# Avokadoen/zig_vulkan

Hardware: AMD Instinct MI355X
Metric: Mrays/s at 1920x1080 on 512^3 brickmap (8^3 bricks, primary + shadow, 1 spp); achieved % of HBM roofline (higher is better)
Workload: dtype f32

## Files before the change

### bindings/vrt_hip.zig

```

const std = @import("std");

pub const Ctx = opaque {};
pub const Grid = opaque {};
pub const Vox = opaque {};
pub const Benchmark = opaque {};

pub const Status = enum(c_int) {
    ok = 0,
    invalid_arg = -1,
    oom = -2,
    out_of_range = -3,
    hip = -4,
    no_device = -5,
    state = -6,
    rccl = -7,
    vox_invalid_id = -100,
    vox_expected_size_header = -101,
    vox_expected_xyzi_header = -102,
    vox_expected_rgba_header = -103,
    vox_unexpected_version = -104,
    vox_invalid_file_content = -105,
    vox_multiple_pack_chunks = -106,
    _,
// ... 151 lines not shown

pub const TUNE_NO_SKIP_TO_BOX: u32 = 1 << 0;
pub const TUNE_NO_PATH_BRICK_LDS: u32 = 1 << 1;
pub const TUNE_NO_PATH_HALFBLOCKS: u32 = 1 << 2;
pub const TUNE_PATH_EAGER_START: u32 = 1 << 3;
pub const TUNE_DIST_NO_BROADCAST: u32 = 1 << 4;
pub const TUNE_NO_CELL_OCCUPANCY: u32 = 1 << 5;
pub const TUNE_NO_START_SHORTCUT: u32 = 1 << 6;
pub const TUNE_PATH_AHEAD: u32 = 1 << 7;
pub const TUNE_PATH_DISTANCE: u32 = 1 << 8;
pub const TUNE_NO_PATH_DILATED: u32 = 1 << 9;
pub const TUNE_NO_PATH_GRID_EXIT: u32 = 1 << 10;
pub const TUNE_PATH_BLOCKS64: u32 = 1 << 11;
pub const TUNE_PATH_TWO_AHEAD: u32 = 1 << 12;
pub const TUNE_NO_PATH_POOL: u32 = 1 << 13;
pub const TUNE_NO_SMALL_FRAME_SPLIT: u32 = 1 << 14;
pub const TUNE_NO_BOUNCE_WAVE_GROUPS: u32 = 1 << 15;
pub const TUNE_NO_SAMPLE_UNITS: u32 = 1 << 16;
pub const TUNE_NO_DEFERRED_MATERIAL: u32 = 1 << 17;
pub const TUNE_NO_CELL_MATERIAL: u32 = 1 << 18;
pub const TUNE_GRID_EXIT_ANY_BOX: u32 = 1 << 19;
pub const TUNE_NO_BOUNCE_AUTOTUNE: u32 = 1 << 20;
pub const TUNE_PRESENT_OWN_STREAM: u32 = 1 << 21;

pub const GridConfig = extern struct {
    brick_alloc: u64 = 0,
    base_t: f32 = 0.01,
    min_point: [3]f32 = .{ 0, 0, 0 },
    scale: f32 = 1.0,
    brick_dimension: u32 = 4,
};

pub const CameraConfig = extern struct {
    viewport_height: f32 = 2,
    origin: [3]f32 = .{ 0, 0, 0 },
    samples_per_pixel: i32 = 2,
    max_bounce: i32 = 2,
};

pub const SunConfig = extern struct {
    enabled: u32 = 1,
    color: [3]f32 = .{ 1, 1.1, 1 },
    radius: f32 = 5,
    sun_distance: f32 = 1000,
};

// ... 149 lines not shown
```

### include/vrt_hip.h

```cpp
#ifndef VRT_HIP_H
#define VRT_HIP_H

#include <stdint.h>

#ifdef __cplusplus
extern "C" {
#endif

#define VRT_ABI_VERSION 4u

enum {
    VRT_OK = 0,
    VRT_E_INVALID_ARG = -1,
    VRT_E_OOM = -2,
    VRT_E_OUT_OF_RANGE = -3,
    VRT_E_HIP = -4,
    VRT_E_NO_DEVICE = -5,
    VRT_E_STATE = -6,
    VRT_E_RCCL = -7
};

typedef enum vrt_buffer_id {
    VRT_BUF_GRID_STATE = 0,
    VRT_BUF_MATERIALS = 1,
// ... 68 lines not shown

#define VRT_TUNE_NO_SKIP_TO_BOX     (1u << 0)
#define VRT_TUNE_NO_PATH_BRICK_LDS  (1u << 1)
#define VRT_TUNE_NO_PATH_HALFBLOCKS (1u << 2)
#define VRT_TUNE_PATH_EAGER_START   (1u << 3)
#define VRT_TUNE_DIST_NO_BROADCAST  (1u << 4)
#define VRT_TUNE_NO_CELL_OCCUPANCY  (1u << 5)
#define VRT_TUNE_NO_START_SHORTCUT  (1u << 6)
#define VRT_TUNE_PATH_AHEAD          (1u << 7)
#define VRT_TUNE_PATH_DISTANCE       (1u << 8)
#define VRT_TUNE_NO_PATH_DILATED     (1u << 9)
#define VRT_TUNE_NO_PATH_GRID_EXIT   (1u << 10)
#define VRT_TUNE_PATH_BLOCKS64        (1u << 11)
#define VRT_TUNE_PATH_TWO_AHEAD       (1u << 12)
#define VRT_TUNE_NO_PATH_POOL         (1u << 13)
#define VRT_TUNE_NO_SMALL_FRAME_SPLIT (1u << 14)
#define VRT_TUNE_NO_BOUNCE_WAVE_GROUPS (1u << 15)
#define VRT_TUNE_NO_SAMPLE_UNITS     (1u << 16)
#define VRT_TUNE_NO_DEFERRED_MATERIAL (1u << 17)
#define VRT_TUNE_NO_CELL_MATERIAL     (1u << 18)
#define VRT_TUNE_GRID_EXIT_ANY_BOX    (1u << 19)
#define VRT_TUNE_NO_BOUNCE_AUTOTUNE   (1u << 20)
#define VRT_TUNE_PRESENT_OWN_STREAM   (1u << 21)
#define VRT_TUNE_ALL                0x3FFFFFu

typedef struct vrt_ctx vrt_ctx;

int vrt_create(const vrt_config *cfg, vrt_ctx **out);

void vrt_destroy(vrt_ctx *ctx);

int vrt_upload(vrt_ctx *ctx, vrt_buffer_id id, uint64_t byte_offset, const void *src, uint64_t nbytes);

uint64_t vrt_buffer_size(const vrt_ctx *ctx, vrt_buffer_id id);

int vrt_upload_device(vrt_ctx *ctx, vrt_buffer_id id, uint64_t byte_offset, const void *dev_src, uint64_t nbytes);

int vrt_dispatch(vrt_ctx *ctx, const vrt_camera_device *camera, const vrt_sun_device *sun);
int vrt_wait(vrt_ctx *ctx);

int vrt_reserve_samples(vrt_ctx *ctx, uint32_t max_samples_per_pixel);

int vrt_dispatch_repeat(vrt_ctx *ctx, const vrt_camera_device *camera, const vrt_sun_device *sun, uint32_t frames);

int vrt_dispatch_timed(vrt_ctx *ctx, const vrt_camera_device *camera, const vrt_sun_device *sun, uint32_t frames, float *ms_per_frame);

int vrt_read_rgba8(vrt_ctx *ctx, void *dst, uint64_t nbytes);
// ... 178 lines not shown
```

### zig_vulkan_amd/_lib.py

```python
from __future__ import annotations

import ctypes as C
import os

_HERE = os.path.dirname(os.path.abspath(__file__))
LIB_PATH = os.environ.get("VRT_HIP_LIB") or os.path.join(_HERE, "libvrt_hip.so")

VRT_ABI_VERSION = 4

VRT_OK = 0
VRT_E_INVALID_ARG = -1
VRT_E_OOM = -2
VRT_E_OUT_OF_RANGE = -3
VRT_E_HIP = -4
VRT_E_NO_DEVICE = -5
VRT_E_STATE = -6
VRT_E_RCCL = -7

ERROR_NAMES = {
    VRT_E_INVALID_ARG: "VRT_E_INVALID_ARG",
    VRT_E_OOM: "VRT_E_OOM",
    VRT_E_OUT_OF_RANGE: "VRT_E_OUT_OF_RANGE",
    VRT_E_HIP: "VRT_E_HIP",
    VRT_E_NO_DEVICE: "VRT_E_NO_DEVICE",
    VRT_E_STATE: "VRT_E_STATE",
    VRT_E_RCCL: "VRT_E_RCCL",
}

TUNE_NO_SKIP_TO_BOX, TUNE_NO_PATH_BRICK_LDS, TUNE_NO_PATH_HALFBLOCKS, TUNE_PATH_EAGER_START, TUNE_DIST_NO_BROADCAST = 1, 2, 4, 8, 16
TUNE_NO_CELL_OCCUPANCY, TUNE_NO_START_SHORTCUT, TUNE_PATH_AHEAD, TUNE_PATH_DISTANCE, TUNE_NO_PATH_DILATED, TUNE_NO_PATH_GRID_EXIT, TUNE_PATH_BLOCKS64, TUNE_PATH_TWO_AHEAD = 32, 64, 128, 256, 512, 1024, 2048, 4096
TUNE_NO_SMALL_FRAME_SPLIT = 16384
TUNE_NO_BOUNCE_WAVE_GROUPS = 32768
TUNE_NO_SAMPLE_UNITS = 65536
TUNE_NO_DEFERRED_MATERIAL = 131072
TUNE_NO_CELL_MATERIAL = 262144
TUNE_GRID_EXIT_ANY_BOX = 524288
TUNE_NO_BOUNCE_AUTOTUNE = 1048576
TUNE_PRESENT_OWN_STREAM = 2097152
TUNE_NO_PATH_POOL = 8192

BUF_GRID_STATE, BUF_MATERIALS, BUF_BRICK_STATUS, BUF_BRICK_INDEX, BUF_BRICK_OCCUPANCY, BUF_BRICK_START_INDEX, BUF_MATERIAL_INDEX = range(7)
BUF_COUNT = 7


class VrtError(RuntimeError):
    def __init__(self, code: int, message: str):
        super().__init__(f"{ERROR_NAMES.get(code, code)}: {message}")
        self.code = code


class GridState(C.Structure):
    _fields_ = [
        ("voxel_dim_x", C.c_uint32), ("voxel_dim_y", C.c_uint32), ("voxel_dim_z", C.c_uint32),
        ("dim_x", C.c_uint32), ("dim_y", C.c_uint32), ("dim_z", C.c_uint32),
        ("padding1", C.c_uint32), ("padding2", C.c_uint32),
        ("min_point_base_t", C.c_float * 4),
        ("max_point_scale", C.c_float * 4),
    ]


class Material(C.Structure):
# ... 241 lines not shown
```

### zig_vulkan_amd/csrc/vrt_api.hip

```cpp
#include <hip/hip_runtime.h>
#include <algorithm>
#include <cstdio>
#include <cstdlib>
#include <cstring>
#include <mutex>
#include <new>
#include <string>
#include <thread>
#include "host_brick_grid.hpp"
#include "vrt_ctx.h"

using namespace vrt_impl;

namespace {
thread_local std::string g_create_error;
}

namespace vrt_impl {

int fail(vrt_ctx *ctx, int code, const std::string &msg) {
    if (ctx) ctx->err = msg;
    else g_create_error = msg;
    return code;
}

void free_ctx(vrt_ctx *c) {
    if (!c) return;
    DeviceGuard dg(c->device);
    if (c->stream) (void)hipStreamSynchronize(c->stream);
    query_release(c);
    dist_destroy(c);
    c->res.release_all();
// ... 444 lines not shown
        const bool cnt = cfg->enable_counters != 0;
        if (!c->kernel || !c->kernel_lockstep || !c->kernel_single || !c->kernel_single1 ||
            (cnt && (!c->product[0] || !c->product[1] || !c->product[2]))) {
            free_ctx(c);
#ifdef VRT_DEV_VARIANTS
            return fail(nullptr, VRT_E_INVALID_ARG, "no kernel for this configuration");
#else
            return fail(nullptr, VRT_E_INVALID_ARG, "no kernel for this kernel_variant in the product build of libvrt_hip (development variants: make dev)");
#endif
        }
        auto any_kernel = [&](auto pred) {
            const vrt::KernelFn fns[12] = {c->kernel, c->kernel_lockstep, c->kernel_single, c->kernel_single1, c->product[0], c->product[1], c->product[2],
                                           c->kernel_grid_exit, c->product_grid_exit, c->kernel_grid_exit_path, c->product_grid_exit_path, c->bounce_auto};
            for (vrt::KernelFn fn : fns) {
                const vrt::KernelEntry *e = fn ? vrt::kernel_entry_of(fn) : nullptr;
                if (e && pred(*e)) return true;
            }
            return false;
        };
        if (any_kernel([](const vrt::KernelEntry &e) { return !e.path && e.mode == vrt::kStatusBytes; })) {
            const size_t status_bytes_size = (size_t)((cells + 31u) / 32u) * 32u + 64u;
            VRT_CREATE_HIP(c->res.device(&c->d_status_bytes, status_bytes_size));
            VRT_CREATE_HIP(hipMemsetAsync(c->d_status_bytes, 0, status_bytes_size, c->stream));
        }
        if (any_kernel([](const vrt::KernelEntry &e) { return e.path && (e.half || e.dil); })) {
            const size_t bytes_hb = (size_t)(cells / 32u) * 4u + 64u;
            VRT_CREATE_HIP(c->res.device(&c->d_status_halfblocks, bytes_hb));
            VRT_CREATE_HIP(hipMemsetAsync(c->d_status_halfblocks, 0, bytes_hb, c->stream));
        }
        if (any_kernel([](const vrt::KernelEntry &e) { return e.path && e.dist; })) {
            VRT_CREATE_HIP(c->res.device(&c->d_cell_distance, (size_t)cells + 64u));
            VRT_CREATE_HIP(hipMemsetAsync(c->d_cell_distance, 0xFF, (size_t)cells + 64u, c->stream));
        }
        const uint64_t by_cell_bytes = cells * (bits / 8u);
        const bool lds_walk = cfg->brick_dimension == 8u && !(cfg->tuning_flags & VRT_TUNE_NO_PATH_BRICK_LDS);
        size_t mem_free = 0, mem_total = 0;
        if (hipMemGetInfo(&mem_free, &mem_total) != hipSuccess) mem_free = 0;
        const bool persistent = any_kernel([](const vrt::KernelEntry &e) { return e.path != 0; });
        const bool lockstep_bounce = any_kernel([](const vrt::KernelEntry &e) { return e.path == 0 && e.shade == 0 && !e.count; }) &&
                                     by_cell_bytes <= (64ull << 20) && cells * bits <= (1ull << 32);
        if ((persistent || lockstep_bounce) && !(cfg->tuning_flags & VRT_TUNE_NO_CELL_OCCUPANCY) &&
            by_cell_bytes <= (2ull << 30) && by_cell_bytes + 64u <= mem_free / 4u && (lds_walk || cells * bits <= (1ull << 32))) {
            if (c->res.device(&c->d_cell_occupancy, by_cell_bytes + 64u) != hipSuccess) {
                (void)hipGetLastError();
                c->d_cell_occupancy = nullptr;
            } else {
// ... 77 lines not shown
        dev_knob("VRT_DEV_POOL_TRANS_THR", p.pool_trans_thr);
        dev_knob("VRT_DEV_POOL_WALK_MIN", p.pool_walk_min);
#endif
    }
    p.width = cfg->width;
    p.height = cfg->height;
    p.tiles_x = sh.tiles_x;
    p.pool_tiles_x_magic = sh.tiles_x > 1u ? (uint32_t)((1ull << 32) / sh.tiles_x) + 1u : 0u;
    p.tiles_y = sh.tiles_y;
    p.shard_rank = sh.shard_rank;
    p.shard_count = sh.shard_count;
    p.owned_tiles = sh.owned_tiles;
    if (c->own.period) {
        p.own_period = c->own.period;
        p.own_count = c->own.count[sh.shard_rank];
        uint32_t k = 0;
        for (uint32_t j = 0; j < c->own.period; j++)
            if (c->own.owner[j] == sh.shard_rank) p.own_slots[k++] = (uint8_t)j;
    }
    p.status_words = (uint32_t)((cells + 31u) / 32u);
    p.occupancy_words = (uint32_t)(c->dsize[VRT_BUF_BRICK_OCCUPANCY] / 4u);
    p.status_blocks = static_cast<const uint2 *>(c->d_status_blocks);
    p.cell_bounds = c->d_cell_bounds;
    p.status_bytes = c->d_status_bytes;
    p.status_halfblocks = c->d_status_halfblocks;
    p.cell_distance = c->d_cell_distance;
    p.cell_occupancy = c->d_cell_occupancy;
    p.cell_occupancy_lockstep = (c->d_cell_occupancy && c->cell_occupancy_lockstep) ? 1u : 0u;
    p.start_is_slot = c->d_start_is_slot;
    p.materials_plain = c->d_materials_plain;
    p.cell_material = c->d_cell_material;
    p.status_cells = (uint32_t)cells;
    p.tile_order = c->tile_order;
    p.sched_extra = c->sched_extra;
    p.sched_units = c->sched_cap[0];
    if (p.tile_order == 7u) {
        p.tile_order = 5u;
        c->sched_period = (cfg->kernel_variant >> 28) ? (1u << (cfg->kernel_variant >> 28)) : 32u;
        VRT_CREATE_HIP(c->res.event(&c->ev_sched, hipEventDisableTiming));
        VRT_CREATE_HIP(c->res.event(&c->ev_b_sched, hipEventDisableTiming));
    }
    p.tile_cost = c->d_tile_cost;
    p.tile_schedule = c->d_tile_schedule;
    p.wave_groups = (cfg->kernel_variant >> 20) & 0x1u;
    p.wave_groups_bounce = (cfg->tuning_flags & VRT_TUNE_NO_BOUNCE_WAVE_GROUPS) ? 0u : 1u;
    {
// ... 206 lines not shown
```

### zig_vulkan_amd/csrc/vrt_ctx.h

```cpp
#pragma once
#include <hip/hip_runtime.h>
#include <chrono>
#include <string>
#include <vector>
#include "vrt_internal.h"
#include "vrt_kernels.h"

namespace vrt {
KernelFn select_trace_kernel(int brick_dimension, bool counters, uint32_t variant, int shade);
KernelFn path_kernel_halfblock_twin(KernelFn fn);
KernelFn path_kernel_ahead_twin(KernelFn fn);
KernelFn path_kernel_dist_twin(KernelFn fn);
KernelFn path_kernel_dilated_twin(KernelFn fn, int kind);
int path_kernel_dilated_kind(KernelFn fn);
bool is_path_halfblock_kernel(KernelFn fn);
const char *kernel_name_of(KernelFn fn);
uint32_t resolve_variant(uint32_t variant);
size_t trace_lds_bytes(const TraceParams &p, uint32_t variant);
hipError_t launch_trace(KernelFn fn, const TraceParams &p, size_t lds_bytes, hipStream_t stream, uint32_t frames = 1);
bool is_path_kernel(KernelFn fn);
hipError_t launch_schedule(const uint32_t *cost, uint32_t *snap, const uint32_t *prev_order, uint32_t *order, uint32_t n, uint32_t extra_max, uint32_t extra, uint32_t wave_slots,
                           hipStream_t stream);
hipError_t launch_assemble_rgb(const void *gathered, void *frame, uint32_t width, uint32_t height, uint32_t tiles_x, uint32_t shard_count,
                               uint32_t tiles_per_rank, const TileOwnership &own, hipStream_t stream, uint32_t frames, uint32_t frame_src_stride_bytes);
hipError_t launch_build_status_blocks(const TraceParams &p, uint32_t dim_x, uint32_t dim_y, uint32_t dim_z, hipStream_t stream);
hipError_t launch_build_status_bytes(const TraceParams &p, hipStream_t stream);
hipError_t launch_build_status_halfblocks(const TraceParams &p, uint32_t dim_x, uint32_t dim_y, uint32_t dim_z, hipStream_t stream);
hipError_t launch_build_cell_distance(const TraceParams &p, uint32_t dim_x, uint32_t dim_y, uint32_t dim_z, hipStream_t stream);
hipError_t launch_build_cell_bounds(const TraceParams &p, uint32_t dim_x, uint32_t dim_y, uint32_t dim_z, hipStream_t stream);
hipError_t launch_build_cell_occupancy(const TraceParams &p, uint32_t brick_dimension, uint64_t brick_alloc, uint64_t cell_lo, uint64_t cell_hi, uint64_t slot_lo,
                                       uint64_t slot_hi, hipStream_t stream);
hipError_t launch_build_cell_material(const TraceParams &p, uint32_t brick_dimension, uint64_t brick_alloc, uint64_t cell_lo, uint64_t cell_hi, uint64_t slot_lo,
                                      uint64_t slot_hi, uint64_t mat_lo, uint64_t mat_hi, hipStream_t stream);
hipError_t launch_check_start_is_slot(const TraceParams &p, uint32_t brick_dimension, uint64_t brick_alloc, hipStream_t stream);
hipError_t launch_check_materials_plain(const TraceParams &p, uint32_t count, hipStream_t stream);
hipError_t launch_denoise(const void *img, int W, int H, int samples, float bias, float mult, float tol, int out_w, int out_h, void *out_u8,
                          void *out_f32, hipStream_t stream);
hipError_t launch_assemble(const void *gathered, void *frame, uint32_t bytes_per_pixel, uint32_t width, uint32_t height, uint32_t tiles_x,
                           uint32_t shard_count, uint32_t tiles_per_rank, const TileOwnership &own, hipStream_t stream, uint32_t frames = 1,
                           uint32_t frame_src_stride_pixels = 0);

class Resources {
public:
    template <class T> hipError_t device(T **out, size_t bytes) {
        void *p = nullptr;
        const hipError_t e = hipMalloc(&p, bytes);
        if (e == hipSuccess) {
            items_.push_back({Kind::Device, p});
            *out = static_cast<T *>(p);
        }
        return e;
    }
// ... 79 lines not shown
    int last_slot = 0;
    void *dbuf[VRT_BUF_COUNT] = {};
    uint64_t dsize[VRT_BUF_COUNT] = {};
    uint8_t *target8 = nullptr;
    float *target32f = nullptr;
    uint64_t target_pixels = 0;
    vrt::DeviceCounters *d_counters = nullptr;
    uint32_t *d_tile_cost = nullptr, *d_tile_schedule = nullptr;
    uint32_t sched_period = 0, sched_since = 0, sched_cur = 0;
    bool order_auto = false;
    uint32_t bounce_variant = 0;
    uint32_t single_variant = 0;
    uint32_t tile_order = 0, sched_extra = 0, sched_stride = 0, wave_slots = 0;
    uint32_t sched_cap[2] = {0, 0}, sched_slots[2] = {0, 0}, sched_mode = 0;
    uint64_t sched_seq = 0, b_seen_sched = 0;
    hipEvent_t ev_sched = nullptr, ev_b_sched = nullptr;
    bool b_sched_recorded = false;
    void *d_denoised8 = nullptr, *d_denoised32f = nullptr;
    Dist *dist = nullptr;
    uint32_t denoised_w = 0, denoised_h = 0;
    hipStream_t denoised_stream = nullptr;
    void *d_status_blocks = nullptr;
    int *d_cell_bounds = nullptr;
    int *h_cell_bounds = nullptr;
    hipEvent_t ev_bounds = nullptr;
    bool bounds_pending = false, box_is_grid = false;
    vrt::KernelFn kernel_grid_exit = nullptr, product_grid_exit = nullptr, kernel_grid_exit_path = nullptr, product_grid_exit_path = nullptr;
    uint8_t *d_status_bytes = nullptr;
    uint8_t *d_cell_distance = nullptr;
    uint32_t *d_status_halfblocks = nullptr;
    bool cell_occupancy_lockstep = false;
    uint8_t *d_cell_occupancy = nullptr;
    uint32_t *d_start_is_slot = nullptr;
    bool occupancy_dirty = true;
    uint64_t occ_cell_lo = 0, occ_cell_hi = ~0ull, occ_slot_lo = 0, occ_slot_hi = 0;
    uint8_t *d_cell_material = nullptr;
    bool cell_material_dirty = true;
    uint64_t cm_cell_lo = 0, cm_cell_hi = ~0ull, cm_slot_lo = 0, cm_slot_hi = 0, cm_mat_lo = 0, cm_mat_hi = 0;
    uint32_t *d_materials_plain = nullptr;
    bool materials_dirty = true;
    bool start_dirty = true;
    vrt::TileOwnership own{};
    bool status_dirty = true;
    bool grid_uploaded = false;
    hipModule_t query_module = nullptr;
    hipFunction_t query_fn = nullptr;
// ... 107 lines not shown
```

### zig_vulkan_amd/csrc/vrt_frame.hip

```cpp
#include <hip/hip_runtime.h>
#include <algorithm>
#include <cstring>
#include <string>
#include <vector>
#include "vrt_ctx.h"

using namespace vrt_impl;

namespace vrt_impl {

void note_kernel(vrt_ctx *c, vrt::KernelFn fn) {
    if (fn == c->last_fn) return;
    c->last_fn = fn;
    c->kernel_name = std::string(vrt::kernel_name_of(fn)) + c->name_note;
}

int finish_frame(vrt_ctx *c) {
    if (!c->in_flight) return VRT_OK;
    VRT_HIP(c, wait_event(c->ev_stop));
    float ms = 0.0f;
    VRT_HIP(c, hipEventElapsedTime(&ms, c->ev_start, c->ev_stop));
    c->last_ms = (double)ms / (double)(c->timed_frames ? c->timed_frames : 1u);
    c->timing_valid = true;
    c->in_flight = false;
// ... 52 lines not shown
int refresh_derived(vrt_ctx *ctx) {
    const vrt_grid_state &g = ctx->params.grid;
    {
        auto pow2_with_normal_reciprocal = [](float v) {
            uint32_t b;
            std::memcpy(&b, &v, 4);
            const uint32_t e = (b >> 23) & 0xFFu;
            return (b & 0x7FFFFFu) == 0u && e >= 2u && e <= 252u;
        };
        const float gs = g.max_point_scale[3];
        const float vs = gs * (1.0f / (float)ctx->cfg.brick_dimension);
        const bool ok = pow2_with_normal_reciprocal(gs) && pow2_with_normal_reciprocal(vs);
        ctx->params.scale_pow2 = ok ? 1u : 0u;
        ctx->params.inv_grid_scale = ok ? 1.0f / gs : 0.0f;
        ctx->params.inv_voxel_scale = ok ? 1.0f / vs : 0.0f;
    }
    if (g.dim_x != 0 && (g.dim_x != ctx->cfg.dim_x || g.dim_y != ctx->cfg.dim_y || g.dim_z != ctx->cfg.dim_z))
        return fail(ctx, VRT_E_INVALID_ARG, "uploaded grid state has other brick dimensions than the context was created with");
    if (ctx->status_dirty) {
        int rcw = begin_scene_write(ctx);
        if (rcw != VRT_OK) return rcw;
        VRT_HIP(ctx, vrt::launch_build_status_blocks(ctx->params, ctx->cfg.dim_x, ctx->cfg.dim_y, ctx->cfg.dim_z, ctx->stream));
        VRT_HIP(ctx, vrt::launch_build_cell_bounds(ctx->params, ctx->cfg.dim_x, ctx->cfg.dim_y, ctx->cfg.dim_z, ctx->stream));
        if (ctx->kernel_grid_exit || ctx->product_grid_exit || ctx->bounce_auto) {
            if (!ctx->h_cell_bounds) VRT_HIP(ctx, ctx->res.pinned(&ctx->h_cell_bounds, 6 * sizeof(int)));
            if (!ctx->ev_bounds) VRT_HIP(ctx, ctx->res.event(&ctx->ev_bounds, hipEventDisableTiming));
            if (ctx->bounds_pending) VRT_HIP(ctx, hipEventSynchronize(ctx->ev_bounds));
            VRT_HIP(ctx, hipMemcpyAsync(ctx->h_cell_bounds, ctx->d_cell_bounds, 6 * sizeof(int), hipMemcpyDeviceToHost, ctx->stream));
            VRT_HIP(ctx, hipEventRecord(ctx->ev_bounds, ctx->stream));
            ctx->bounds_pending = true;
            ctx->box_is_grid = false;
            ctx->auto_next = 0;
            ctx->auto_decided = ctx->auto_use_pool = false;
        }
        VRT_HIP(ctx, vrt::launch_build_status_bytes(ctx->params, ctx->stream));
        VRT_HIP(ctx, vrt::launch_build_status_halfblocks(ctx->params, ctx->cfg.dim_x, ctx->cfg.dim_y, ctx->cfg.dim_z, ctx->stream));
        VRT_HIP(ctx, vrt::launch_build_cell_distance(ctx->params, ctx->cfg.dim_x, ctx->cfg.dim_y, ctx->cfg.dim_z, ctx->stream));
        rcw = end_scene_write(ctx);
        if (rcw != VRT_OK) return rcw;
        ctx->status_dirty = false;
    }
    if ((ctx->occupancy_dirty && ctx->d_cell_occupancy) || (ctx->start_dirty && ctx->d_start_is_slot) || (ctx->materials_dirty && ctx->d_materials_plain)) {
        int rcw = begin_scene_write(ctx);
        if (rcw != VRT_OK) return rcw;
        if (ctx->occupancy_dirty)
            VRT_HIP(ctx, vrt::launch_build_cell_occupancy(ctx->params, ctx->cfg.brick_dimension, ctx->cfg.brick_alloc, ctx->occ_cell_lo, ctx->occ_cell_hi, ctx->occ_slot_lo,
// ... 354 lines not shown
```

### zig_vulkan_amd/csrc/vrt_internal.h

```cpp
#pragma once
#include <hip/hip_runtime.h>
#include <stdint.h>
#include "../../include/vrt_hip.h"

namespace vrt {

struct PushConstants {
    vrt_camera_device cam;
    vrt_sun_device sun;
};
static_assert(sizeof(vrt_camera_device) == 96, "Camera.Device is 96 bytes (Camera.zig:183-193)");
static_assert(sizeof(vrt_sun_device) == 32, "Sun.Device is 32 bytes (Sun.zig:13-18)");
static_assert(sizeof(PushConstants) == 128, "push constant range is 128 bytes (ComputePipeline.zig:258-272)");
static_assert(sizeof(vrt_grid_state) == 64, "State.Device is 64 bytes (State.zig:60-79)");
static_assert(sizeof(vrt_material) == 20, "Material is 20 bytes (gpu_types.zig:16-32)");

struct DeviceCounters {
    unsigned long long rays, status_loads, bricks_entered, voxel_steps, hits, grid_steps;
    unsigned long long wave_grid_iters, wave_brick_walks, wave_voxel_iters;
};

struct TileOwnership {
    uint32_t period;
    uint32_t ranks;
// ... 6 lines not shown
    vrt_grid_state grid;
    PushConstants pcs[8];
    const vrt_material *materials;
    const uint32_t *brick_status;
    const uint32_t *brick_index;
    const uint8_t *brick_occupancy;
    const uint32_t *brick_start_index;
    const uint8_t *material_index;
    uint8_t *target_rgba8;
    float *target_rgba32f;
    DeviceCounters *counters;
    uint32_t width, height;
    uint32_t batch_target_stride;
    uint32_t tiles_x, tiles_y;
    uint32_t shard_rank, shard_count;
    uint32_t owned_tiles;
    uint32_t own_period, own_count;
    uint8_t own_slots[16];
    uint32_t status_words;
    uint32_t scale_pow2;
    float inv_grid_scale, inv_voxel_scale;
    uint32_t occupancy_words;
    const int *cell_bounds;
    const uint32_t *status_halfblocks;
    const uint8_t *status_bytes;
    uint32_t status_cells;
    const uint8_t *cell_distance;
    const uint8_t *cell_occupancy;
    uint32_t cell_occupancy_lockstep;
    const uint32_t *start_is_slot;
    const uint32_t *materials_plain;
    const uint8_t *cell_material;
    const uint2 *status_blocks;
    uint32_t nbx, nby, nbz;
    uint32_t *tile_cost;
    unsigned long long *wave_timeline;
    const uint32_t *tile_schedule;
    uint32_t tile_stride;
    uint32_t sched_extra;
    uint32_t sched_units;
    uint32_t packed_tiles;
    uint32_t packed_rgb;
    uint32_t brick_batch;
    uint32_t path_brick_batch;
    uint32_t block_threads;
    uint32_t wave_groups;
// ... 46 lines not shown
```

### zig_vulkan_amd/csrc/vrt_trace.hip

```cpp
#include <hip/hip_runtime.h>
#include <cstdlib>
#include <climits>
#include "vrt_internal.h"
#include "vrt_kernels.h"

namespace vrt {

__global__ __launch_bounds__(256) void vrt_build_status_blocks(const uint32_t *__restrict__ status, uint2 *__restrict__ out, uint32_t dim_x,
                                                               uint32_t dim_y, uint32_t dim_z, uint32_t nbx, uint32_t nby, uint32_t nbz) {
    const uint32_t nblocks = nbx * nby * nbz;
    const uint32_t b = blockIdx.x * 256u + threadIdx.x;
    uint2 word = make_uint2(0u, 0u);
    if (b < nblocks) {
        const uint32_t bx = b % nbx, bz = (b / nbx) % nbz, by = b / (nbx * nbz);
        for (uint32_t yy = 0; yy < 4u; yy++)
            for (uint32_t zz = 0; zz < 4u; zz++)
                for (uint32_t xx = 0; xx < 4u; xx++) {
                    const uint32_t x = bx * 4u + xx, y = by * 4u + yy, z = bz * 4u + zz;
                    if (x < dim_x && y < dim_y && z < dim_z) {
                        const uint32_t gi = x + dim_x * (z + dim_z * y);
                        const uint32_t bit = (status[gi >> 5] >> (gi & 31u)) & 1u;
                        const uint32_t pos = xx + 4u * zz + 16u * yy;
                        if (pos < 32u) word.x |= bit << pos;
                        else word.y |= bit << (pos - 32u);
                    }
                }
        out[b] = word;
// ... 130 lines not shown
        uint32_t id = 0xFFu;
        if (any != 0ull) {
            const uint32_t leader = (uint32_t)__builtin_ctzll(any);
            const uint32_t m = (uint32_t)__shfl((int)first, (int)leader, 64);
            if (__builtin_amdgcn_ballot_w64(solid && (!same || first != m)) == 0ull) id = m;
        }
        if (lane == 0u) out[cell] = (uint8_t)id;
    }
}

__global__ __launch_bounds__(256) void vrt_check_start_is_slot(const uint32_t *__restrict__ start, uint32_t *__restrict__ flag, uint64_t brick_alloc,
                                                               uint32_t bits) {
    const uint64_t i = (uint64_t)blockIdx.x * 256u + threadIdx.x;
    if (i >= brick_alloc) return;
    const uint32_t v = start[i];
    if (v != 0xFFFFFFFFu && (uint64_t)(v & 0x7FFFFFFFu) != i * bits) *flag = 0u;
}

__global__ __launch_bounds__(256) void vrt_check_materials_plain(const vrt_material *__restrict__ materials, uint32_t *__restrict__ flag, uint32_t count) {
    const uint32_t i = blockIdx.x * 256u + threadIdx.x;
    if (i < count && materials[i].type == 3u ) *flag = 0u;
}

__global__ __launch_bounds__(256) void vrt_build_cell_bounds(const uint32_t *__restrict__ status, int *__restrict__ bounds, uint32_t words,
                                                             uint32_t cells, uint32_t dim_x, uint32_t dim_z) {
    const uint32_t wi = blockIdx.x * 256u + threadIdx.x;
    if (wi >= words) return;
    uint32_t bits = status[wi];
    if (wi == words - 1u && (cells & 31u)) bits &= (1u << (cells & 31u)) - 1u;
    if (bits == 0u) return;
    int m[6] = {INT_MIN, INT_MIN, INT_MIN, INT_MIN, INT_MIN, INT_MIN};
    while (bits) {
        const uint32_t b = (uint32_t)__builtin_ctz(bits);
        bits &= bits - 1u;
        const uint32_t i = wi * 32u + b;
        const int x = (int)(i % dim_x), z = (int)((i / dim_x) % dim_z), y = (int)(i / (dim_x * dim_z));
        m[0] = max(m[0], -x), m[1] = max(m[1], -y), m[2] = max(m[2], -z);
        m[3] = max(m[3], x), m[4] = max(m[4], y), m[5] = max(m[5], z);
    }
#pragma unroll
    for (int k = 0; k < 6; k++) atomicMax(&bounds[k], m[k]);
}

constexpr uint32_t kScheduleBuckets = 8u;
constexpr uint32_t kSplitBuckets = 8u;
constexpr uint32_t kAllBuckets = kScheduleBuckets + kSplitBuckets;
__global__ __launch_bounds__(1024) void vrt_schedule_kernel(const uint32_t *__restrict__ cost, uint32_t *__restrict__ snap,
                                                            const uint32_t *prev_order, uint32_t *order, uint32_t n, uint32_t extra_max,
                                                            uint32_t extra, uint32_t wave_slots) {
    __shared__ uint32_t s_max, s_nsplit, s_longest;
    __shared__ unsigned long long s_total;
    __shared__ uint32_t wave_total[kAllBuckets][16];
    __shared__ uint32_t class_total[kAllBuckets];
    const uint32_t tid = threadIdx.x, lane = tid & 63u, wv = tid >> 6;
    uint32_t *state = snap + n;
    const uint32_t row = (n + extra_max + 7u) >> 3;
    if (tid == 0) {
        s_max = 0u;
        s_nsplit = 0u;
        s_longest = 0u;
        s_total = 0ull;
    }
    __syncthreads();
    uint32_t m = 0u, ml = 0u;
// ... 452 lines not shown
    uint32_t *flag = const_cast<uint32_t *>(p.start_is_slot);
    const hipError_t e = hipMemsetD32Async(reinterpret_cast<hipDeviceptr_t>(flag), 1, 1, stream);
    if (e != hipSuccess) return e;
    VRT_LAUNCH(vrt_check_start_is_slot, dim3((uint32_t)((brick_alloc + 255u) / 256u)), dim3(256), 0, stream, p.brick_start_index, flag, brick_alloc,
                       brick_dimension * brick_dimension * brick_dimension);
    return hipGetLastError();
}

hipError_t launch_check_materials_plain(const TraceParams &p, uint32_t count, hipStream_t stream) {
    if (!p.materials_plain) return hipSuccess;
    uint32_t *flag = const_cast<uint32_t *>(p.materials_plain);
    const hipError_t e = hipMemsetD32Async(reinterpret_cast<hipDeviceptr_t>(flag), 1, 1, stream);
    if (e != hipSuccess) return e;
    if (count) VRT_LAUNCH(vrt_check_materials_plain, dim3((count + 255u) / 256u), dim3(256), 0, stream, p.materials, flag, count);
    return hipGetLastError();
}

hipError_t launch_build_cell_bounds(const TraceParams &p, uint32_t dim_x, uint32_t dim_y, uint32_t dim_z, hipStream_t stream) {
    if (!p.cell_bounds) return hipSuccess;
    int *bounds = const_cast<int *>(p.cell_bounds);
    hipError_t e = hipMemsetAsync(bounds, 0x80, 6 * sizeof(int), stream);
    if (e != hipSuccess) return e;
    VRT_LAUNCH(vrt_build_cell_bounds, dim3((p.status_words + 255u) / 256u), dim3(256), 0, stream, p.brick_status, bounds, p.status_words,
                       dim_x * dim_y * dim_z, dim_x, dim_z);
    return hipGetLastError();
}

hipError_t launch_build_status_bytes(const TraceParams &p, hipStream_t stream) {
    if (!p.status_bytes) return hipSuccess;
    VRT_LAUNCH(vrt_build_status_bytes, dim3((p.status_words + 255u) / 256u), dim3(256), 0, stream, p.brick_status,
                       const_cast<uint8_t *>(p.status_bytes), p.status_words, p.status_cells);
    return hipGetLastError();
}

hipError_t launch_build_status_blocks(const TraceParams &p, uint32_t dim_x, uint32_t dim_y, uint32_t dim_z, hipStream_t stream) {
    if (!p.status_blocks) return hipSuccess;
    const uint32_t nblocks = p.nbx * p.nby * p.nbz;
    VRT_LAUNCH(vrt_build_status_blocks, dim3((nblocks + 255u) / 256u), dim3(256), 0, stream, p.brick_status,
                       const_cast<uint2 *>(p.status_blocks), dim_x, dim_y, dim_z, p.nbx, p.nby, p.nbz);
    return hipGetLastError();
}

hipError_t launch_assemble_rgb(const void *gathered, void *frame, uint32_t width, uint32_t height, uint32_t tiles_x, uint32_t shard_count,
                               uint32_t tiles_per_rank, const TileOwnership &own, hipStream_t stream, uint32_t frames, uint32_t frame_src_stride_bytes) {
    if (width % 4u == 0u && (reinterpret_cast<uintptr_t>(frame) & 15u) == 0u && (reinterpret_cast<uintptr_t>(gathered) & 3u) == 0u &&
        frame_src_stride_bytes % 4u == 0u) {
        const dim3 grid4((width / 4u + 63u) / 64u, (height + 3u) / 4u, frames);
// ... 28 lines not shown
```

### zig_vulkan_amd/csrc/vrt_trace_kernels.h

```cpp
#pragma once
#include <hip/hip_runtime.h>
#include "vrt_internal.h"
#include "vrt_kernels.h"
#include "vrt_math.h"

namespace vrt {

constexpr uint32_t MAT_LAMBERTIAN = 0, MAT_METAL = 1, MAT_DIELECTRIC = 2, MAT_NONE = 3;

struct Ray {
    f3 origin, direction;
    float internal_reflection;
    uint32_t ignore_type_material;
};

struct Hit {
    f3 point, normal;
    float t;
    uint32_t index;
};

template <bool COUNT>
struct Cnt {
    uint32_t rays = 0, status_loads = 0, bricks_entered = 0, voxel_steps = 0, hits = 0, grid_steps = 0;
    uint32_t wave_grid_iters = 0, wave_brick_walks = 0, wave_voxel_iters = 0;
};
template <>
// ... 960 lines not shown
        skipped = true;
    }
}
VRT_DI bool skip_to_box(Walk &w, const RaySetup &s, int span_x, int span_y, int span_z, uint32_t &index, uint32_t stride_x, uint32_t stride_y,
                        uint32_t stride_z, bool &more, int &in_axis, float &t_in) {
    bool skipped = false;
    skip_round<0>(w, s, span_x, index, stride_x, stride_y, stride_z, more, in_axis, t_in, skipped);
    skip_round<1>(w, s, span_y, index, stride_x, stride_y, stride_z, more, in_axis, t_in, skipped);
    skip_round<2>(w, s, span_z, index, stride_x, stride_y, stride_z, more, in_axis, t_in, skipped);
    return skipped;
}

#ifdef VRT_DEV_VARIANTS
#define VRT_DEV_SECTION 6
#include "vrt_trace_kernels_dev.h"
#undef VRT_DEV_SECTION
#endif
VRT_DI float opaque_uniform(float v) {
    asm volatile("" : "+s"(v));
    return v;
}
VRT_DI f3 opaque_uniform3(const float (&v)[3]) { return mk3(opaque_uniform(v[0]), opaque_uniform(v[1]), opaque_uniform(v[2])); }

template <int B, bool COUNT, int MODE, bool BATCH = false, bool SCALAR_ENTRY = false, bool VOXEL = false>
VRT_DI bool grid_hit(const TraceParams &p, const uint32_t *lds_filter, const Ray &r, Hit &hit, Cnt<COUNT> &c, int *voxel = nullptr) {
    static_assert(!VOXEL || ((MODE == kStatusLinearAlways || MODE == kStatusLinearLds || MODE == kStatusBytes) && !COUNT && !BATCH),
                  "voxel coordinates come from the hand-written walk without batching");
    const float t_min = 0.00001f;
    const float t_max = __builtin_inff();
    VRT_COUNT(rays);
    VRT_PROF_BEGIN(tp3);
    RaySetup s;
    VRT_PROF_BEGIN(tp6);
    const bool slab_hit = grid_slab(p, r, t_min, t_max, s);
    VRT_PROF_END(6, tp6);
    if (!slab_hit) return false;

    const f3 g_min = mk3(p.grid.min_point_base_t[0], p.grid.min_point_base_t[1], p.grid.min_point_base_t[2]);
    const float g_scale = p.grid.max_point_scale[3];
    const int dx = (int)p.grid.dim_x, dy = (int)p.grid.dim_y, dz = (int)p.grid.dim_z;

    float global_t_value = s.grid_t_min + 0.0001f * (SCALAR_ENTRY ? opaque_uniform(g_scale) : g_scale);
    const f3 fposition = p.scale_pow2 ? (ray_at(r, global_t_value) - g_min) * p.inv_grid_scale : (ray_at(r, global_t_value) - g_min) / splat3(g_scale);
    Walk w;
    w.side_dist = initial_side_dist(mk3((float)s.sx, (float)s.sy, (float)s.sz), fposition, s.ray_delta());
    const int px = f2i_clamp(__builtin_floorf(fposition.x));
    const int py = f2i_clamp(__builtin_floorf(fposition.y));
    const int pz = f2i_clamp(__builtin_floorf(fposition.z));
    const int zero_budget = dx + dy + dz + 8;
    int lox = 0, loy = 0, loz = 0, hix = dx - 1, hiy = dy - 1, hiz = dz - 1;
    if (!COUNT || p.count_box) {
        if (p.cell_bounds) {
            lox = -p.cell_bounds[0], loy = -p.cell_bounds[1], loz = -p.cell_bounds[2];
            hix = p.cell_bounds[3], hiy = p.cell_bounds[4], hiz = p.cell_bounds[5];
        }
    }
    w.rx = steps_left_box(s.sx, px, lox, hix, zero_budget);
    w.ry = steps_left_box(s.sy, py, loy, hiy, zero_budget);
    w.rz = steps_left_box(s.sz, pz, loz, hiz, zero_budget);
    const int base_x = walk_base_box(s.sx, px, lox, hix), base_y = walk_base_box(s.sy, py, loy, hiy), base_z = walk_base_box(s.sz, pz, loz, hiz);
    w.t_value = 0;

    uint32_t word_index = ~0u;
    uint32_t word_bits = 0;
    uint32_t block_index = ~0u;
    uint2 block_bits = make_uint2(0u, 0u);
    int axis = 3;
    [[maybe_unused]] int hit_axis = 0;

    if (!(global_t_value <= t_max)) return false;
    uint32_t grid_index = (uint32_t)px + (uint32_t)dx * ((uint32_t)pz + (uint32_t)dz * (uint32_t)py);
    const uint32_t stride_x = (uint32_t)s.sx, stride_y = (uint32_t)s.sy * (uint32_t)dx * (uint32_t)dz, stride_z = (uint32_t)s.sz * (uint32_t)dx;

    int stop = 0;
    bool more = (unsigned)px < (unsigned)dx && (unsigned)py < (unsigned)dy && (unsigned)pz < (unsigned)dz && (w.rx | w.ry | w.rz) >= 0;
    [[maybe_unused]] bool skipped = false;
    [[maybe_unused]] float skip_t = 0.0f;
    if ((!COUNT || p.count_box) && p.cell_bounds && p.skip_to_box) {
        VRT_PROF_BEGIN(tp5);
        skipped = skip_to_box(w, s, (int)((uint32_t)hix - (uint32_t)lox), (int)((uint32_t)hiy - (uint32_t)loy), (int)((uint32_t)hiz - (uint32_t)loz), grid_index,
                              stride_x, stride_y, stride_z, more, axis, skip_t);
        w.t_value = skip_t;
        VRT_PROF_END(5, tp5);
    }

    auto cell_occupied = [&]() -> bool {
        VRT_COUNT(grid_steps);
        VRT_COUNT_WAVE(wave_grid_iters);
        if constexpr (MODE == kStatusLinearLds) {
            if constexpr (COUNT) {
                const uint32_t wi = grid_index >> 5;
                if (wi != word_index) {
                    word_index = wi;
                    c.status_loads++;
                }
            }
            return status_bit(lds_word0(grid_index >> 5), grid_index);
        } else if constexpr (MODE == kStatusLinearAlways) {
// ... 239 lines not shown
    } else {
        direction = reflect3(r_in.direction, normal);
        scattered = create_ray(hit.point, direction);
    }
    return true;
}

template <int B, bool COUNT, int MODE, bool SCALAR_ENTRY = false>
VRT_DI f3 ray_color_single(const TraceParams &p, const PushConstants &pc, const uint32_t *lds_filter, const Ray &ray, Cnt<COUNT> &c) {
    const bool sun_enabled = pc.sun.enabled > 0;
    const f3 sun_color = mk3(pc.sun.color[0], pc.sun.color[1], pc.sun.color[2]);
    f3 color = mk3(0, 0, 0);
    int loop_count = 0;
    Hit hit;
    if (pc.cam.max_bounce > 0 && grid_hit<B, COUNT, MODE, false, SCALAR_ENTRY>(p, lds_filter, ray, hit, c)) {
        const uint32_t material = hit.index;
        bool lit = true;
        if (sun_enabled) {
            const f3 sun_position = mk3(pc.sun.position[0], pc.sun.position[1], pc.sun.position[2]);
            const f3 rv = rand_vec3_range(ray.direction.x + ray.direction.z, ray.direction.y + ray.direction.z, -pc.sun.radius,
                                          pc.sun.radius);
            const Ray shadow_ray = create_ray(hit.point, (sun_position + rv) - hit.point);
            Hit shadow_hit;
            lit = !grid_hit<B, COUNT, MODE, false, SCALAR_ENTRY>(p, lds_filter, shadow_ray, shadow_hit, c);
        }
        const vrt_material *m = p.materials + material;
        const uint32_t mtype = m->type;
        const f3 attenuation = mk3(m->albedo_r, m->albedo_g, m->albedo_b);
        loop_count = (mtype <= MAT_DIELECTRIC) ? 1 : 0;
        if (sun_enabled) {
            if (lit) color = color + attenuation * sun_color;
        } else {
            color = color + attenuation;
        }
    }
    if (loop_count == 0) {
        const float t = 0.5f * (ray.direction.y + 1.0f);
        const f3 bg = fma3(splat3(1.0f - t), splat3(1.0f), mk3(0.5f, 0.7f, 1.0f) * t);
        color = color + bg * (sun_enabled ? sun_color : splat3(1.0f));
    }
    return color / (color + splat3(1.0f));
}

template <int B, bool COUNT, int MODE>
VRT_DI f3 ray_color(const TraceParams &p, const PushConstants &pc, const uint32_t *lds_filter, Ray current_ray, Cnt<COUNT> &c) {
    const bool sun_enabled = pc.sun.enabled > 0;
    const f3 sun_color = mk3(pc.sun.color[0], pc.sun.color[1], pc.sun.color[2]);
// ... 259 lines not shown
```

Measured before the change: 34810.

## Add per-column Y-bounds mip pyramid to tighten shadow-ray traversal box

Builds a 2D mip pyramid over the XZ columns of the brick grid, where each entry stores the min and max occupied Y, using two extra build kernel stages. Shadow rays (non-scalar-entry path) look up the four pyramid entries covering their XZ footprint and clamp the Y walk range, and exit immediately when no occupied Y lies in range. The aim is to skip empty grid steps for shadow rays above the terrain. The cost is extra per-ray setup math and four gathered loads, plus a small build pass that runs a single-block reduction.

```diff
diff --git a/bindings/vrt_hip.zig b/bindings/vrt_hip.zig
--- a/bindings/vrt_hip.zig
+++ b/bindings/vrt_hip.zig
@@ -197,6 +197,7 @@
 pub const TUNE_GRID_EXIT_ANY_BOX: u32 = 1 << 19;
 pub const TUNE_NO_BOUNCE_AUTOTUNE: u32 = 1 << 20;
 pub const TUNE_PRESENT_OWN_STREAM: u32 = 1 << 21;
+pub const TUNE_NO_COLUMN_BOUNDS: u32 = 1 << 22;
 
 pub const GridConfig = extern struct {
     brick_alloc: u64 = 0,
diff --git a/include/vrt_hip.h b/include/vrt_hip.h
--- a/include/vrt_hip.h
+++ b/include/vrt_hip.h
@@ -114,7 +114,8 @@
 #define VRT_TUNE_GRID_EXIT_ANY_BOX    (1u << 19)
 #define VRT_TUNE_NO_BOUNCE_AUTOTUNE   (1u << 20)
 #define VRT_TUNE_PRESENT_OWN_STREAM   (1u << 21)
-#define VRT_TUNE_ALL                0x3FFFFFu
+#define VRT_TUNE_NO_COLUMN_BOUNDS    (1u << 22)
+#define VRT_TUNE_ALL                0x7FFFFFu
 
 typedef struct vrt_ctx vrt_ctx;
 
diff --git a/zig_vulkan_amd/_lib.py b/zig_vulkan_amd/_lib.py
--- a/zig_vulkan_amd/_lib.py
+++ b/zig_vulkan_amd/_lib.py
@@ -37,6 +37,7 @@
 TUNE_GRID_EXIT_ANY_BOX = 524288
 TUNE_NO_BOUNCE_AUTOTUNE = 1048576
 TUNE_PRESENT_OWN_STREAM = 2097152
+TUNE_NO_COLUMN_BOUNDS = 4194304
 TUNE_NO_PATH_POOL = 8192
 
 BUF_GRID_STATE, BUF_MATERIALS, BUF_BRICK_STATUS, BUF_BRICK_INDEX, BUF_BRICK_OCCUPANCY, BUF_BRICK_START_INDEX, BUF_MATERIAL_INDEX = range(7)
diff --git a/zig_vulkan_amd/csrc/vrt_api.hip b/zig_vulkan_amd/csrc/vrt_api.hip
--- a/zig_vulkan_amd/csrc/vrt_api.hip
+++ b/zig_vulkan_amd/csrc/vrt_api.hip
@@ -8,6 +8,7 @@
 #include <string>
 #include <thread>
 #include "host_brick_grid.hpp"
+#include "vrt_colbounds.h"
 #include "vrt_ctx.h"
 
 using namespace vrt_impl;
@@ -498,6 +499,15 @@
             const size_t status_bytes_size = (size_t)((cells + 31u) / 32u) * 32u + 64u;
             VRT_CREATE_HIP(c->res.device(&c->d_status_bytes, status_bytes_size));
             VRT_CREATE_HIP(hipMemsetAsync(c->d_status_bytes, 0, status_bytes_size, c->stream));
+        }
+        if (!(cfg->tuning_flags & VRT_TUNE_NO_COLUMN_BOUNDS) && any_kernel([](const vrt::KernelEntry &e) { return !e.path; })) {
+            c->col_side = vrt::colb_side(cfg->dim_x, cfg->dim_z);
+            c->col_wide = cfg->dim_y > 256u;
+            const size_t bytes = (size_t)vrt::colb_entries(c->col_side) * (c->col_wide ? 4u : 2u);
+            VRT_CREATE_HIP(c->res.device(&c->d_col_bounds, bytes));
+            const size_t entries = vrt::colb_entries(c->col_side);
+            VRT_CREATE_HIP(c->col_wide ? hipMemsetD32Async(reinterpret_cast<hipDeviceptr_t>(c->d_col_bounds), 0xFFFF0000u, entries, c->stream)
+                                       : hipMemsetD16Async(reinterpret_cast<hipDeviceptr_t>(c->d_col_bounds), 0xFF00u, entries, c->stream));
         }
         if (any_kernel([](const vrt::KernelEntry &e) { return e.path && (e.half || e.dil); })) {
             const size_t bytes_hb = (size_t)(cells / 32u) * 4u + 64u;
@@ -621,6 +631,9 @@
     p.occupancy_words = (uint32_t)(c->dsize[VRT_BUF_BRICK_OCCUPANCY] / 4u);
     p.status_blocks = static_cast<const uint2 *>(c->d_status_blocks);
     p.cell_bounds = c->d_cell_bounds;
+    p.col_bounds = c->d_col_bounds;
+    p.col_side = c->col_side;
+    p.col_wide = c->col_wide ? 1u : 0u;
     p.status_bytes = c->d_status_bytes;
     p.status_halfblocks = c->d_status_halfblocks;
     p.cell_distance = c->d_cell_distance;
diff --git a/zig_vulkan_amd/csrc/vrt_colbounds.h b/zig_vulkan_amd/csrc/vrt_colbounds.h
--- /dev/null
+++ b/zig_vulkan_amd/csrc/vrt_colbounds.h
@@ -0,0 +1,54 @@
+#pragma once
+#include <stdint.h>
+
+#if defined(__HIPCC__)
+#define VRT_HD __host__ __device__ inline
+#else
+#define VRT_HD inline
+#endif
+
+namespace vrt {
+
+VRT_HD uint32_t colb_side(uint32_t dim_x, uint32_t dim_z) {
+    const uint32_t m = dim_x > dim_z ? dim_x : dim_z;
+    uint32_t n = 2u;
+    while (n < m) n <<= 1;
+    return n;
+}
+VRT_HD uint32_t colb_entries(uint32_t n) { return (n + n / 2u) * n; }
+VRT_HD uint32_t colb_levels(uint32_t n) { return 32u - (uint32_t)__builtin_clz(n); }
+VRT_HD uint32_t colb_index(uint32_t n, uint32_t k, uint32_t bx, uint32_t bz) {
+    const uint32_t pitch = n + n / 2u;
+    return k == 0u ? bx + pitch * bz : (n + bx) + pitch * (n - (n >> (k - 1u)) + bz);
+}
+
+struct ColRange {
+    int x0, x1, z0, z1;
+};
+VRT_HD float colb_min(float a, float b) { return b < a ? b : a; }
+VRT_HD float colb_max(float a, float b) { return a < b ? b : a; }
+VRT_HD int colb_clampi(int v, int lo, int hi) { return v < lo ? lo : (v > hi ? hi : v); }
+VRT_HD ColRange column_range(float fx, float fz, float ex, float ez, const int lo[3], const int hi[3], int dim_x, int dim_z) {
+    const float x_lo = colb_max((float)colb_clampi(lo[0], 0, dim_x - 1), 0.0f), x_hi = (float)colb_clampi(hi[0], 0, dim_x - 1);
+    const float z_lo = colb_max((float)colb_clampi(lo[2], 0, dim_z - 1), 0.0f), z_hi = (float)colb_clampi(hi[2], 0, dim_z - 1);
+    ColRange c;
+    c.x0 = (int)colb_min(colb_max(colb_min(fx, ex) - 1.0f, x_lo), x_hi);
+    c.x1 = (int)colb_max(colb_min(colb_max(fx, ex) + 1.0f, x_hi), (float)c.x0);
+    c.z0 = (int)colb_min(colb_max(colb_min(fz, ez) - 1.0f, z_lo), z_hi);
+    c.z1 = (int)colb_max(colb_min(colb_max(fz, ez) + 1.0f, z_hi), (float)c.z0);
+    return c;
+}
+VRT_HD uint32_t colb_level(const ColRange &c) {
+    const uint32_t d = (uint32_t)(c.x1 - c.x0) | (uint32_t)(c.z1 - c.z0);
+    return d == 0u ? 0u : 32u - (uint32_t)__builtin_clz(d);
+}
+VRT_HD void colb_query_indices(uint32_t n, const ColRange &c, uint32_t idx[4]) {
+    const uint32_t k = colb_level(c);
+    const uint32_t bx0 = (uint32_t)c.x0 >> k, bx1 = (uint32_t)c.x1 >> k, bz0 = (uint32_t)c.z0 >> k, bz1 = (uint32_t)c.z1 >> k;
+    idx[0] = colb_index(n, k, bx0, bz0);
+    idx[1] = colb_index(n, k, bx1, bz0);
+    idx[2] = colb_index(n, k, bx0, bz1);
+    idx[3] = colb_index(n, k, bx1, bz1);
+}
+
+}
diff --git a/zig_vulkan_amd/csrc/vrt_ctx.h b/zig_vulkan_amd/csrc/vrt_ctx.h
--- a/zig_vulkan_amd/csrc/vrt_ctx.h
+++ b/zig_vulkan_amd/csrc/vrt_ctx.h
@@ -28,6 +28,7 @@
 hipError_t launch_build_status_halfblocks(const TraceParams &p, uint32_t dim_x, uint32_t dim_y, uint32_t dim_z, hipStream_t stream);
 hipError_t launch_build_cell_distance(const TraceParams &p, uint32_t dim_x, uint32_t dim_y, uint32_t dim_z, hipStream_t stream);
 hipError_t launch_build_cell_bounds(const TraceParams &p, uint32_t dim_x, uint32_t dim_y, uint32_t dim_z, hipStream_t stream);
+hipError_t launch_build_col_bounds(const TraceParams &p, uint32_t dim_x, uint32_t dim_y, uint32_t dim_z, hipStream_t stream);
 hipError_t launch_build_cell_occupancy(const TraceParams &p, uint32_t brick_dimension, uint64_t brick_alloc, uint64_t cell_lo, uint64_t cell_hi, uint64_t slot_lo,
                                        uint64_t slot_hi, hipStream_t stream);
 hipError_t launch_build_cell_material(const TraceParams &p, uint32_t brick_dimension, uint64_t brick_alloc, uint64_t cell_lo, uint64_t cell_hi, uint64_t slot_lo,
@@ -153,6 +154,9 @@
     hipStream_t denoised_stream = nullptr;
     void *d_status_blocks = nullptr;
     int *d_cell_bounds = nullptr;
+    void *d_col_bounds = nullptr;
+    uint32_t col_side = 0;
+    bool col_wide = false;
     int *h_cell_bounds = nullptr;
     hipEvent_t ev_bounds = nullptr;
     bool bounds_pending = false, box_is_grid = false;
diff --git a/zig_vulkan_amd/csrc/vrt_frame.hip b/zig_vulkan_amd/csrc/vrt_frame.hip
--- a/zig_vulkan_amd/csrc/vrt_frame.hip
+++ b/zig_vulkan_amd/csrc/vrt_frame.hip
@@ -98,6 +98,7 @@
         if (rcw != VRT_OK) return rcw;
         VRT_HIP(ctx, vrt::launch_build_status_blocks(ctx->params, ctx->cfg.dim_x, ctx->cfg.dim_y, ctx->cfg.dim_z, ctx->stream));
         VRT_HIP(ctx, vrt::launch_build_cell_bounds(ctx->params, ctx->cfg.dim_x, ctx->cfg.dim_y, ctx->cfg.dim_z, ctx->stream));
+        VRT_HIP(ctx, vrt::launch_build_col_bounds(ctx->params, ctx->cfg.dim_x, ctx->cfg.dim_y, ctx->cfg.dim_z, ctx->stream));
         if (ctx->kernel_grid_exit || ctx->product_grid_exit || ctx->bounce_auto) {
             if (!ctx->h_cell_bounds) VRT_HIP(ctx, ctx->res.pinned(&ctx->h_cell_bounds, 6 * sizeof(int)));
             if (!ctx->ev_bounds) VRT_HIP(ctx, ctx->res.event(&ctx->ev_bounds, hipEventDisableTiming));
diff --git a/zig_vulkan_amd/csrc/vrt_internal.h b/zig_vulkan_amd/csrc/vrt_internal.h
--- a/zig_vulkan_amd/csrc/vrt_internal.h
+++ b/zig_vulkan_amd/csrc/vrt_internal.h
@@ -52,6 +52,9 @@
     float inv_grid_scale, inv_voxel_scale;
     uint32_t occupancy_words;
     const int *cell_bounds;
+    const void *col_bounds;
+    uint32_t col_side;
+    uint32_t col_wide;
     const uint32_t *status_halfblocks;
     const uint8_t *status_bytes;
     uint32_t status_cells;
diff --git a/zig_vulkan_amd/csrc/vrt_trace.hip b/zig_vulkan_amd/csrc/vrt_trace.hip
--- a/zig_vulkan_amd/csrc/vrt_trace.hip
+++ b/zig_vulkan_amd/csrc/vrt_trace.hip
@@ -3,6 +3,7 @@
 #include <climits>
 #include "vrt_internal.h"
 #include "vrt_kernels.h"
+#include "vrt_colbounds.h"
 
 namespace vrt {
 
@@ -179,9 +180,57 @@
     if (i < count && materials[i].type == 3u ) *flag = 0u;
 }
 
-__global__ __launch_bounds__(256) void vrt_build_cell_bounds(const uint32_t *__restrict__ status, int *__restrict__ bounds, uint32_t words,
-                                                             uint32_t cells, uint32_t dim_x, uint32_t dim_z) {
+template <typename T, int S>
+__device__ void col_bounds_level0(const uint32_t *__restrict__ status, void *bounds, uint32_t i, uint32_t n, uint32_t dim_x, uint32_t dim_y,
+                                  uint32_t dim_z) {
+    if (i >= n * n) return;
+    const uint32_t x = i % n, z = i / n;
+    uint32_t lo = (1u << S) - 1u, hi = 0u;
+    if (x < dim_x && z < dim_z) {
+        const uint32_t layer = dim_x * dim_z;
+        uint32_t c = x + dim_x * z;
+        for (uint32_t y = 0; y < dim_y; y++, c += layer) {
+            if ((status[c >> 5] >> (c & 31u)) & 1u) {
+                lo = min(lo, y);
+                hi = y;
+            }
+        }
+    }
+    static_cast<T *>(bounds)[colb_index(n, 0u, x, z)] = (T)(lo | (hi << S));
+}
+template <typename T, int S>
+__device__ void col_bounds_up(void *bounds, uint32_t n) {
+    T *out = static_cast<T *>(bounds);
+    const uint32_t mask = (1u << S) - 1u;
+    for (uint32_t k = 1u, m = n >> 1; m != 0u; k++, m >>= 1) {
+        for (uint32_t i = threadIdx.x; i < m * m; i += 256u) {
+            const uint32_t bx = i % m, bz = i / m;
+            uint32_t lo = mask, hi = 0u;
+#pragma unroll
+            for (uint32_t j = 0; j < 4u; j++) {
+                const uint32_t e = out[colb_index(n, k - 1u, 2u * bx + (j & 1u), 2u * bz + (j >> 1))];
+                lo = min(lo, e & mask);
+                hi = max(hi, e >> S);
+            }
+            out[colb_index(n, k, bx, bz)] = (T)(lo | (hi << S));
+        }
+        __syncthreads();
+    }
+}
+
+__global__ __launch_bounds__(256) void vrt_build_cell_bounds(const uint32_t *__restrict__ status, void *bounds, uint32_t words, uint32_t cells,
+                                                             uint32_t dim_x, uint32_t dim_y, uint32_t dim_z, uint32_t stage, uint32_t n, uint32_t wide) {
     const uint32_t wi = blockIdx.x * 256u + threadIdx.x;
+    if (stage == 1u) {
+        if (wide) col_bounds_level0<uint32_t, 16>(status, bounds, wi, n, dim_x, dim_y, dim_z);
+        else col_bounds_level0<uint16_t, 8>(status, bounds, wi, n, dim_x, dim_y, dim_z);
+        return;
+    }
+    if (stage == 2u) {
+        if (wide) col_bounds_up<uint32_t, 16>(bounds, n);
+        else col_bounds_up<uint16_t, 8>(bounds, n);
+        return;
+    }
     if (wi >= words) return;
     uint32_t bits = status[wi];
     if (wi == words - 1u && (cells & 31u)) bits &= (1u << (cells & 31u)) - 1u;
@@ -196,7 +245,7 @@
         m[3] = max(m[3], x), m[4] = max(m[4], y), m[5] = max(m[5], z);
     }
 #pragma unroll
-    for (int k = 0; k < 6; k++) atomicMax(&bounds[k], m[k]);
+    for (int k = 0; k < 6; k++) atomicMax(&static_cast<int *>(bounds)[k], m[k]);
 }
 
 constexpr uint32_t kScheduleBuckets = 8u;
@@ -695,7 +744,20 @@
     hipError_t e = hipMemsetAsync(bounds, 0x80, 6 * sizeof(int), stream);
     if (e != hipSuccess) return e;
     VRT_LAUNCH(vrt_build_cell_bounds, dim3((p.status_words + 255u) / 256u), dim3(256), 0, stream, p.brick_status, bounds, p.status_words,
-                       dim_x * dim_y * dim_z, dim_x, dim_z);
+                       dim_x * dim_y * dim_z, dim_x, dim_y, dim_z, 0u, 0u, 0u);
+    return hipGetLastError();
+}
+
+hipError_t launch_build_col_bounds(const TraceParams &p, uint32_t dim_x, uint32_t dim_y, uint32_t dim_z, hipStream_t stream) {
+    if (!p.col_bounds) return hipSuccess;
+    void *bounds = const_cast<void *>(p.col_bounds);
+    const uint32_t n = p.col_side;
+    VRT_LAUNCH(vrt_build_cell_bounds, dim3((n * n + 255u) / 256u), dim3(256), 0, stream, p.brick_status, bounds, p.status_words,
+                       dim_x * dim_y * dim_z, dim_x, dim_y, dim_z, 1u, n, p.col_wide);
+    const hipError_t e = hipGetLastError();
+    if (e != hipSuccess) return e;
+    VRT_LAUNCH(vrt_build_cell_bounds, dim3(1), dim3(256), 0, stream, p.brick_status, bounds, p.status_words, dim_x * dim_y * dim_z, dim_x, dim_y,
+                       dim_z, 2u, n, p.col_wide);
     return hipGetLastError();
 }
 
diff --git a/zig_vulkan_amd/csrc/vrt_trace_kernels.h b/zig_vulkan_amd/csrc/vrt_trace_kernels.h
--- a/zig_vulkan_amd/csrc/vrt_trace_kernels.h
+++ b/zig_vulkan_amd/csrc/vrt_trace_kernels.h
@@ -3,6 +3,7 @@
 #include "vrt_internal.h"
 #include "vrt_kernels.h"
 #include "vrt_math.h"
+#include "vrt_colbounds.h"
 
 namespace vrt {
 
@@ -1009,7 +1010,7 @@
 }
 VRT_DI f3 opaque_uniform3(const float (&v)[3]) { return mk3(opaque_uniform(v[0]), opaque_uniform(v[1]), opaque_uniform(v[2])); }
 
-template <int B, bool COUNT, int MODE, bool BATCH = false, bool SCALAR_ENTRY = false, bool VOXEL = false>
+template <int B, bool COUNT, int MODE, bool BATCH = false, bool SCALAR_ENTRY = false, bool VOXEL = false, bool COLS = false>
 VRT_DI bool grid_hit(const TraceParams &p, const uint32_t *lds_filter, const Ray &r, Hit &hit, Cnt<COUNT> &c, int *voxel = nullptr) {
     static_assert(!VOXEL || ((MODE == kStatusLinearAlways || MODE == kStatusLinearLds || MODE == kStatusBytes) && !COUNT && !BATCH),
                   "voxel coordinates come from the hand-written walk without batching");
@@ -1041,6 +1042,28 @@
             lox = -p.cell_bounds[0], loy = -p.cell_bounds[1], loz = -p.cell_bounds[2];
             hix = p.cell_bounds[3], hiy = p.cell_bounds[4], hiz = p.cell_bounds[5];
         }
+        if (COLS && p.col_bounds) {
+            const int blo[3] = {lox, loy, loz}, bhi[3] = {hix, hiy, hiz};
+            const float u_exit = (s.grid_t_max - global_t_value) * __builtin_amdgcn_rcpf(g_scale);
+            const ColRange cr = column_range(fposition.x, fposition.z, fposition.x + u_exit * r.direction.x, fposition.z + u_exit * r.direction.z, blo, bhi, dx, dz);
+            uint32_t idx[4];
+            colb_query_indices(p.col_side, cr, idx);
+            uint32_t e[4];
+            if (p.col_wide) {
+                const uint32_t *t = static_cast<const uint32_t *>(p.col_bounds);
+#pragma unroll
+                for (int j = 0; j < 4; j++) e[j] = t[idx[j]];
+            } else {
+                const uint16_t *t = static_cast<const uint16_t *>(p.col_bounds);
+#pragma unroll
+                for (int j = 0; j < 4; j++) {
+                    const uint32_t v = t[idx[j]];
+                    e[j] = (v & 0xFFu) | ((v >> 8) << 16);
+                }
+            }
+            loy = max(loy, (int)min(min(e[0] & 0xFFFFu, e[1] & 0xFFFFu), min(e[2] & 0xFFFFu, e[3] & 0xFFFFu)));
+            hiy = min(hiy, (int)max(max(e[0] >> 16, e[1] >> 16), max(e[2] >> 16, e[3] >> 16)));
+        }
     }
     w.rx = steps_left_box(s.sx, px, lox, hix, zero_budget);
     w.ry = steps_left_box(s.sy, py, loy, hiy, zero_budget);
@@ -1060,7 +1083,7 @@
     const uint32_t stride_x = (uint32_t)s.sx, stride_y = (uint32_t)s.sy * (uint32_t)dx * (uint32_t)dz, stride_z = (uint32_t)s.sz * (uint32_t)dx;
 
     int stop = 0;
-    bool more = (unsigned)px < (unsigned)dx && (unsigned)py < (unsigned)dy && (unsigned)pz < (unsigned)dz && (w.rx | w.ry | w.rz) >= 0;
+    bool more = (unsigned)px < (unsigned)dx && (unsigned)py < (unsigned)dy && (unsigned)pz < (unsigned)dz && (w.rx | w.ry | w.rz) >= 0 && loy <= hiy;
     [[maybe_unused]] bool skipped = false;
     [[maybe_unused]] float skip_t = 0.0f;
     if ((!COUNT || p.count_box) && p.cell_bounds && p.skip_to_box) {
@@ -1346,7 +1369,7 @@
                                           pc.sun.radius);
             const Ray shadow_ray = create_ray(hit.point, (sun_position + rv) - hit.point);
             Hit shadow_hit;
-            lit = !grid_hit<B, COUNT, MODE, false, SCALAR_ENTRY>(p, lds_filter, shadow_ray, shadow_hit, c);
+            lit = !grid_hit<B, COUNT, MODE, false, SCALAR_ENTRY, false, !SCALAR_ENTRY>(p, lds_filter, shadow_ray, shadow_hit, c);
         }
         const vrt_material *m = p.materials + material;
         const uint32_t mtype = m->type;
```

New measurement: 34810 (median of 6 runs). About the same (+0.0%).
